# Boulder-Computer-Architecture-Lab/shrewd

Measured on AMD Instinct MI355X. Metric: fault-injection trials/sec (whole node), higher is better.
Workload: dtype int64; 1 GPU; crc32 (RV64, 64618 golden insts), 100000 single-bit x1..x31+pc trials per GPU per step; trials_per_gpu=100000, seed=0x5eed0002, structures=x1-x31,pc, burst=1, lanes_per_wave=32, parallelism=trial-sharded x1, RCCL histogram all-reduce

## Files before the change

### include/fi_debug.h

```cpp
#ifndef SHREWD_FI_DEBUG_H
#define SHREWD_FI_DEBUG_H
#include "fi_engine.h"
#ifdef __cplusplus
extern "C" {
#endif
fi_status fi_debug_decode(fi_engine *e, const uint32_t *raws, uint64_t n, void *out);
fi_status fi_debug_stats(fi_engine *e, uint64_t *out64);
fi_status fi_debug_softfp(int op, int fmt, int rm, const uint64_t *a, const uint64_t *b, const uint64_t *c,
                          uint64_t n, uint64_t *out, uint32_t *fl, int on_device);
fi_status fi_debug_waves(fi_engine *e, uint64_t *out, uint64_t n_waves);
fi_status fi_debug_dispatch_ms(fi_engine *e, float *ms, uint32_t cap, uint32_t *n);
fi_status fi_debug_dispatch_span_ms(fi_engine *e, float *ms, uint32_t cap, uint32_t *n);
fi_status fi_debug_dispatch_kinds(fi_engine *e, uint32_t *kinds, uint32_t cap, uint32_t *n);
fi_status fi_debug_epochs(fi_engine *e, uint32_t *out16);
fi_status fi_debug_golden_trace(fi_engine *e, void *pre_out, uint64_t pre_cap, uint64_t *n_pre, uint32_t *trace_out,
                                uint64_t trace_cap, uint64_t *n_trace, uint64_t *text_lo);
fi_status fi_debug_translate(const void *pre, uint64_t n_pre, uint64_t text_lo, const uint32_t *trace,
                             uint64_t n_trace, char *out, uint64_t cap, uint64_t *len);
fi_status fi_debug_loop_est(const void *pre, uint64_t n_pre, uint64_t text_lo, const uint32_t *trace,
                            uint64_t n_trace, void *out, uint64_t cap, uint64_t *n);
fi_status fi_debug_translation(fi_engine *e, char *buf, uint64_t cap, uint64_t *len);
fi_status fi_debug_jit_compile(const char *body, const char *arch, void *code, uint64_t cap, uint64_t *len,
                               char *err, uint64_t err_cap);
fi_status fi_debug_jit_build(const char *body, const char *arch, int part, int use_cache, uint64_t *len,
                             int *cached, char *err, uint64_t err_cap);

typedef struct {
    uint64_t regs[32];
    uint64_t left;
    uint32_t lp_cnt, lp_m, lp_n;
    uint32_t lp_ld[4][3];
    uint32_t pad;
} fi_debug_loop;
typedef struct {
    int32_t verdict;
    uint32_t body_proof;
    uint64_t k, fva;
} fi_debug_loop_out;
fi_status fi_debug_loop_outcome(fi_engine *e, const fi_debug_loop *in, uint64_t n, fi_debug_loop_out *out);
#ifdef __cplusplus
}
// ... 3 lines not shown
```

### include/fi_engine.h

```cpp
#ifndef SHREWD_FI_ENGINE_H
#define SHREWD_FI_ENGINE_H

#ifndef __HIPCC_RTC__
#include <stddef.h>
#include <stdint.h>
#endif

#ifdef __cplusplus
extern "C" {
#endif

typedef int32_t fi_status;
#define FI_OK 0
#define FI_E_ARG -1
#define FI_E_NODEVICE -2
#define FI_E_HIP -3
#define FI_E_ELF -4
#define FI_E_STATE -5
#define FI_E_GOLDEN -6

#define FI_MASKED 0
#define FI_SDC 1
#define FI_CRASH 2
#define FI_HANG 3
// ... 69 lines not shown
    uint32_t flags;
    uint32_t epoch_iters;
    uint32_t lanes_per_wave;
    uint32_t resume_lanes;
    uint32_t epochs;
} fi_config;
#define FI_CFG_NO_SNAPSHOT_START 1u
#define FI_CFG_NO_EARLY_EXIT 2u
#define FI_CFG_NO_TRANSLATE 4u
#define FI_CFG_NO_EPOCHS 8u
#define FI_CFG_PACK_RUNS 16u
#define FI_CFG_FIXED_RESUME 32u
#define FI_CFG_NO_SOLO 64u
#define FI_CFG_SOLO_ALL 128u
#define FI_CFG_SIMT 256u
#define FI_CFG_NO_FORWARD 512u
#define FI_CFG_NO_SDC_EXIT 1024u
#define FI_CFG_NO_REDO 2048u
#define FI_CFG_NO_ODD_KERNEL 4096u
#define FI_CFG_JIT_NO_CACHE 8192u
#define FI_CFG_NO_HANG_PROOF 16384u
#define FI_CFG_NO_OVERFLOW 32768u
#define FI_CFG_NO_LOOP_ORDER 65536u

typedef struct {
    uint64_t ninst, ncycles;
    uint32_t exit_code, pad;
    uint64_t stdout_len, stderr_len;
    uint64_t fetch_bytes, data_bytes;
    uint64_t snapshots, snapshot_interval;
    uint64_t snapshot_frames;
    uint64_t translated_blocks;
    uint64_t translated_insts;
    uint64_t translate_us;
} fi_golden_info;

typedef struct {
    uint64_t counts[FI_N_STRUCT][64][FI_N_CLASS];
    uint64_t crash_sub[16];
    uint64_t escape_sub[8];
    uint64_t trials;
    uint64_t guest_insts;
    uint64_t fetch_bytes;
    uint64_t data_bytes;
    uint64_t cow_pages;
    uint64_t device_insts;
// ... 172 lines not shown
```

### shrewd_amd/csrc/fi_engine.cpp

```cpp
#include <hip/hip_runtime.h>

#include <algorithm>
#include <atomic>
#include <chrono>
#include <condition_variable>
#include <memory>
#include <mutex>
#include <thread>
#include <cstdarg>
#include <cstdio>
#include <cstdlib>
#include <cstring>
#include <map>
#include <random>
#include <string>
#include <vector>

#include "fi_capture.h"
#include "fi_checkpoint.h"
#include "fi_debug.h"
#include "fi_site_draw.h"
#include "fi_tick.h"
#include "fi_tick_map.h"
#include "fi_types.h"
// ... 24 lines not shown
                       const unsigned long long *stats, hipStream_t st);
hipError_t launch_hist_stats(const unsigned long long *stats, fi_histogram *h, hipStream_t st);
hipError_t sort_pairs_bytes(uint64_t n, size_t &bytes);
hipError_t launch_pack_runs(const uint64_t *keys, const uint32_t *cnt, uint64_t cap, uint32_t *wrange,
                            uint32_t *n_waves, hipStream_t st);
hipError_t launch_redo_collect(const fi_outcome *out, uint64_t n, uint32_t *idx, uint32_t *cnt,
                               unsigned long long *stats, hipStream_t st);
hipError_t launch_redo_gather(const fi_site *sites, const uint32_t *idx, uint64_t n, fi_site *rsites, uint64_t *keys,
                              uint32_t *perm, hipStream_t st);
hipError_t launch_redo_scatter(const uint32_t *idx, uint64_t n, const fi_outcome *rout, fi_outcome *out,
                               hipStream_t st);
hipError_t launch_capture_init(uint8_t *rows, uint64_t n, uint32_t stride, uint32_t cap, const uint8_t *gold,
                               uint64_t glen, hipStream_t st);
hipError_t launch_capture_finish(uint8_t *rows, uint64_t n, uint32_t stride, uint32_t cap, const fi_stream_len *lens,
                                 uint32_t err, hipStream_t st);
hipError_t launch_surv_keys(const LaneSave *save, const uint32_t *list, const uint32_t *cnt, uint64_t cap,
                            uint64_t text_lo, uint64_t *keys, uint32_t *vals, uint32_t *n_odd, uint32_t solo,
                            uint64_t golden_ninst, uint32_t nb, const LoopEst *loops, uint32_t n_loops,
                            uint64_t hang_cap, hipStream_t st);
hipError_t launch_odd_split(const uint32_t *cnt, const uint32_t *n_odd, uint32_t *split, uint32_t grid,
                            hipStream_t st);
std::string translate_blocks(const std::vector<PreInst> &pre, uint64_t text_lo, const std::vector<uint32_t> &trace,
                             const std::vector<uint64_t> &extra_pcs, std::vector<uint32_t> &leaders_out,
                             uint32_t &n_insts, bool odd_streams, std::vector<LoopEst> *loops_out = nullptr);
std::vector<fi_issue_op> issue_ops_from_trace(const std::vector<PreInst> &pre, const std::vector<uint32_t> &trace);
std::string jit_compile(const std::string &body, const char *arch, std::vector<char> &code, bool &cached, int part,
                        bool use_cache);
bool jit_has_odd(const std::string &body);
bool jit_parallel_ok();
hipError_t sort_pairs(void *tmp, size_t bytes, const uint64_t *kin, uint64_t *kout, const uint32_t *vin,
                      uint32_t *vout, uint64_t n, int end_bit, hipStream_t st);
}

using namespace fi;

static constexpr uint32_t kDefaultLanes = 32;
static constexpr uint32_t kPreTail = 4;
static constexpr uint32_t kDefaultResumeLanes = 8;
static constexpr uint64_t kJitWindowChunk = 131072;

struct JitJob {
    std::string body, arch;
    bool odd = false;
    bool use_cache = true;
    std::vector<char> code[3];
    std::string err;
    bool cached = true;
// ... 1152 lines not shown
            HIPCHK(hipMalloc(&e->d_fw_off, 33 * 4));
            HIPCHK(hipMalloc(&e->d_fw_ev, std::max<size_t>(ev.size(), 1) * 4));
            HIPCHK(hipMemcpy(e->d_fw_off, off.data(), 33 * 4, hipMemcpyHostToDevice));
            if (!ev.empty()) HIPCHK(hipMemcpy(e->d_fw_ev, ev.data(), ev.size() * 4, hipMemcpyHostToDevice));
            e->fw_ok = true;
        }
    }
    st = upload_snaps(e);
    if (st) return st;
    st = build_mem_index(e, mev, live_ok && n_mem <= mem_cap);
    if (st) return st;
    e->golden_unmapped = stats[62] != 0;
    tick_prepare(e, mev, !trace.empty() && n_mem <= mem_cap);

    free_tx(e);
    if (e->cfg.flags & FI_CFG_NO_TRANSLATE) e->tx_status = "disabled (FI_CFG_NO_TRANSLATE)";
    else if (!e->pre_ok) e->tx_status = "golden run rewrites its text";
    else if (!live_ok || trace.empty()) e->tx_status = "golden trace unavailable";
    else {
        const std::vector<uint64_t> pcs;
        std::vector<uint32_t> leaders;
        std::vector<LoopEst> loops;
        uint32_t n_tx = 0;
        std::string body = translate_blocks(pre, e->text_lo, trace, pcs, leaders, n_tx, true, &loops);
        if (n_tx > 24000) {
            leaders.clear();
            loops.clear();
            body = translate_blocks(pre, e->text_lo, trace, pcs, leaders, n_tx, false, &loops);
        }
        if (!loops.empty() && !(e->cfg.flags & FI_CFG_NO_LOOP_ORDER)) {
            HIPCHK(hipMalloc(&e->d_loops, loops.size() * sizeof(LoopEst)));
            HIPCHK(hipMemcpy(e->d_loops, loops.data(), loops.size() * sizeof(LoopEst), hipMemcpyHostToDevice));
            e->n_loops = (uint32_t)loops.size();
        }
        e->tx_body = body;
        hipDeviceProp_t prop;
        HIPCHK(hipGetDeviceProperties(&prop, e->dev));
        if (const char *dump = getenv("SHREWD_FI_DUMP_TX")) {
            if (FILE *f = fopen(dump, "w")) { fputs(body.c_str(), f); fclose(f); }
        }
        if (leaders.empty()) {
            e->tx_status = "nothing to translate (no code run twice)";
        } else if (n_tx > 24000) {
            e->tx_status = "translation too large";
        } else {
            auto j = std::make_shared<JitJob>();
            j->body = body;
            j->arch = prop.gcnArchName;
            j->odd = jit_has_odd(body);
            j->use_cache = !(e->cfg.flags & FI_CFG_JIT_NO_CACHE);
            for (uint32_t h : leaders) pre[h & 0x7FFFFFFFu].flags |= (h >> 31) ? kPreOddLeader : kPreLeader;
// ... 869 lines not shown
    if (trace_out) memcpy(trace_out, e->g_trace.data(), std::min<uint64_t>(trace_cap, e->g_trace.size()) * 4);
    if (n_pre) *n_pre = e->g_pre.size();
    if (n_trace) *n_trace = e->g_trace.size();
    if (text_lo) *text_lo = e->text_lo;
    return FI_OK;
}

fi_status fi_debug_loop_est(const void *pre, uint64_t n_pre, uint64_t text_lo, const uint32_t *trace,
                            uint64_t n_trace, void *out, uint64_t cap, uint64_t *n) {
    if (!pre || !trace) return FI_E_ARG;
    std::vector<PreInst> p((const PreInst *)pre, (const PreInst *)pre + n_pre);
    std::vector<uint32_t> t(trace, trace + n_trace), leaders;
    std::vector<LoopEst> loops;
    uint32_t n_tx = 0;
    (void)translate_blocks(p, text_lo, t, {}, leaders, n_tx, true, &loops);
    static_assert(sizeof(LoopEst) == 16, "LoopEst is 16 bytes (fi_debug.h)");
    if (out) memcpy(out, loops.data(), std::min<uint64_t>(cap, loops.size()) * sizeof(LoopEst));
    if (n) *n = loops.size();
    return FI_OK;
}

fi_status fi_debug_translate(const void *pre, uint64_t n_pre, uint64_t text_lo, const uint32_t *trace,
                             uint64_t n_trace, char *out, uint64_t cap, uint64_t *len) {
    if (!pre || !trace) return FI_E_ARG;
    std::vector<PreInst> p((const PreInst *)pre, (const PreInst *)pre + n_pre);
    std::vector<uint32_t> t(trace, trace + n_trace);
    std::vector<uint32_t> leaders;
    uint32_t n_tx = 0;
    const std::string body = translate_blocks(p, text_lo, t, {}, leaders, n_tx, true);
    if (out && cap) {
        const uint64_t n = std::min<uint64_t>(cap - 1, body.size());
        memcpy(out, body.data(), n);
        out[n] = 0;
    }
    if (len) *len = body.size();
    return FI_OK;
}

fi_status fi_debug_translation(fi_engine *e, char *buf, uint64_t cap, uint64_t *len) {
    if (!e) return FI_E_ARG;
    if (buf && cap) {
        const uint64_t n = std::min<uint64_t>(cap - 1, e->tx_body.size());
        memcpy(buf, e->tx_body.data(), n);
        buf[n] = 0;
    }
    if (len) *len = e->tx_body.size();
    return FI_OK;
}

fi_status fi_debug_stats(fi_engine *e, uint64_t *out64) {
    if (!e || !out64) return FI_E_ARG;
    HIPCHK(hipStreamSynchronize(e->stream));
// ... 105 lines not shown
```

### shrewd_amd/csrc/fi_translate.cpp

```cpp
#include <cstdlib>
#include <cctype>
#include <cstdarg>
#include <cstdio>
#include <algorithm>
#include <cstring>
#include <map>
#include <set>
#include <unordered_map>
#include <string>
#include <vector>

#include "fi_types.h"
#include "rv64_isa.h"

namespace fi {

namespace {

struct Gen {
    const std::vector<PreInst> &pre;
    uint64_t text_lo;
    const std::set<uint32_t> &leaders;
    const std::set<uint32_t> &executed;
    std::string out;
// ... 272 lines not shown
            }
            if (top) entries.insert(header);
            headers.insert(header);
            for (uint32_t v : comp) chain[v].push_back(header);
            auto inner = removed;
            for (uint32_t v : comp) inner.insert({v, header});
            run(comp, false, inner);
        }
    }
};

struct Block {
    uint32_t h0;
    std::vector<uint32_t> insts;
    bool term;
    uint64_t opc = 0;
    std::vector<uint64_t> opcs;
};

}

std::string translate_blocks(const std::vector<PreInst> &pre, uint64_t text_lo, const std::vector<uint32_t> &trace,
                             const std::vector<uint64_t> &extra_pcs, std::vector<uint32_t> &leaders_out,
                             uint32_t &n_insts, bool odd_streams, std::vector<LoopEst> *loops_out) {
    std::set<uint32_t> executed, leaders;
    auto valid = [&](uint32_t h) { return h < pre.size() && (pre[h].flags & kPreValid); };
    std::unordered_map<uint32_t, uint32_t> runs;
    for (size_t i = 0; i < trace.size(); i++) {
        const uint32_t h = trace[i] & 0x7FFFFFFFu;
        if (valid(h)) runs[h]++;
    }
    for (size_t i = 0; i < trace.size(); i++) {
        const uint32_t h = trace[i] & 0x7FFFFFFFu;
        if (!valid(h) || runs[h] < 2) continue;
        executed.insert(h);
        const bool is_ecall = trace[i] & 0x80000000u;
        if (i == 0) leaders.insert(h);
        if (i + 1 < trace.size()) {
            const uint32_t nh = trace[i + 1] & 0x7FFFFFFFu;
            if (is_ecall || nh != h + pre[h].len / 2u) leaders.insert(nh);
        }
    }
    for (auto it = leaders.begin(); it != leaders.end();) {
        if (!executed.count(*it)) it = leaders.erase(it);
        else ++it;
    }
    for (uint32_t h : executed) {
// ... 148 lines not shown
            const Cls k = ocls(pc);
            if (k == C_BR || k == C_JAL || k == C_JALR) { b.term = true; break; }
            pc += pre[okey(pc)].len;
        }
        blocks.push_back(b);
    }
    bool cur_odd = false;
    bool oddon = false;
    std::string SB = "S_", SD = "S_dispatch", SOB = "SO_";

    enum Edge { E_DIRECT, E_DISPATCH, E_OUT };
    auto edge = [&](uint32_t from, uint64_t pc) {
        uint32_t t;
        if (!hof(pc, t)) return E_OUT;
        return S.exits.count({from, t}) ? E_DISPATCH : E_DIRECT;
    };

    Gen g{pre, text_lo, leaders, executed, {}};
    Gen so{pre, text_lo, leaders, executed, {}};
    Gen sq{pre, text_lo, leaders, executed, {}};
    Gen sc{pre, text_lo, leaders, executed, {}};
    constexpr uint32_t kSiteCaches = 8;
    uint32_t n_sites = 0;
    n_insts = 0;
    auto hex = [](uint64_t v) {
        char b[32];
        snprintf(b, sizeof b, "0x%llxULL", (unsigned long long)v);
        return std::string(b);
    };
    auto wgo = [&](uint32_t from, uint64_t pc) {
        const Edge k = edge(from, pc);
        uint32_t t = 0;
        hof(pc, t);
        if (k == E_DIRECT) return "goto B_" + std::to_string(t) + ";";
        return "{ spc = " + hex(pc) + (k == E_DISPATCH ? "; goto tx_dispatch; }" : "; goto tx_out; }");
    };
    const char *cold = "SCOLD";
    auto sgo = [&](uint32_t from, uint64_t pc) {
        if (oddon && (pc & 1))
            return olead.count(pc) ? "goto " + SOB + std::to_string((uint32_t)((pc - text_lo) >> 1)) + ";"
                                   : "{ spc = " + hex(pc) + "; goto S_out; }";
        if (oddon && cur_odd) return "{ spc = " + hex(pc) + "; goto " + SD + "; }";
        const Edge k = edge(from, pc);
        uint32_t t = 0;
        hof(pc, t);
        if (k == E_DIRECT) return "goto " + SB + std::to_string(t) + ";";
        return "{ spc = " + hex(pc) + (k == E_DISPATCH ? "; goto " + SD + "; }" : "; goto S_out; }");
    };
    struct ProofLoad { uint32_t reg, kind, size, pos; int64_t off; uint64_t span; };
    struct HangProof { uint32_t reg, treg; int step; uint32_t m; std::vector<ProofLoad> loads; bool rel = false; };
    std::map<uint32_t, HangProof> hang_proof;
    struct AVal { int k; uint32_t base; int64_t lo, hi; };
    enum { AV_TOP, AV_CNT, AV_BND, AV_IND };
    const int64_t kAvLim = (int64_t)1 << 40;
    auto av_ok = [&](AVal v) { return v.k == AV_BND && v.lo > -kAvLim && v.hi < kAvLim && v.lo <= v.hi ? v : AVal{AV_TOP, 0, 0, 0}; };
    auto av_add = [&](AVal a, AVal b) -> AVal {
        if (a.k != AV_BND || b.k != AV_BND || (a.base && b.base)) return AVal{AV_TOP, 0, 0, 0};
        return av_ok(AVal{AV_BND, a.base | b.base, a.lo + b.lo, a.hi + b.hi});
    };
    auto av_shl = [&](AVal a, int64_t k) -> AVal {
        if (a.k != AV_BND || a.base || a.lo < 0 || k < 0 || k > 20) return AVal{AV_TOP, 0, 0, 0};
        return av_ok(AVal{AV_BND, 0, a.lo << k, a.hi << k});
    };
    auto av_const = [&](int64_t lo, int64_t hi) { return av_ok(AVal{AV_BND, 0, lo, hi}); };
    for (uint32_t H : S.headers) {
        std::vector<uint32_t> cyc;
        bool nested = false;
        for (const auto &kv : S.chain) {
            const auto pos = std::find(kv.second.begin(), kv.second.end(), H);
            if (pos == kv.second.end()) continue;
            if (pos + 1 != kv.second.end()) nested = true;
            cyc.push_back(kv.first);
        }
        if (nested || cyc.empty()) continue;
        const std::set<uint32_t> in(cyc.begin(), cyc.end());
        std::map<uint32_t, const Block *> bl;
        for (const Block &b : blocks)
            if (b.opc == 0 && in.count(b.h0)) bl[b.h0] = &b;
        if (bl.size() != in.size()) continue;
        bool ok = true;
        uint32_t writes[32] = {0};
        std::map<uint32_t, std::vector<uint32_t>> nx;
        uint32_t n_exit = 0, eblk = 0;
        bool exit_on_taken = false;
        for (const auto &kv : bl) {
            const Block &b = *kv.second;
            if (b.insts.empty()) { ok = false; break; }
            auto to = [&](uint64_t pc, bool taken) {
                uint32_t t;
                if (hof(pc, t) && in.count(t) && !S.exits.count({b.h0, t})) nx[b.h0].push_back(t);
                else { n_exit++; eblk = b.h0; exit_on_taken = taken; }
            };
            for (size_t i = 0; i < b.insts.size() && ok; i++) {
                std::string e;
                uint32_t sz;
                int sx;
                const char *cond;
                const PreInst &p = pre[b.insts[i]];
                const uint64_t pc = text_lo + 2ULL * b.insts[i];
                const Cls k = classify(p, e, sz, sx, cond);
                if (k == C_JALR || k == C_STOP || ((k == C_LOAD || k == C_STORE) && in.size() != 1)) ok = false;
                if ((k == C_ALU || k == C_JAL || k == C_LOAD) && p.rd) writes[p.rd]++;
                if (k == C_BR) { to(pc + (int64_t)p.imm, true); to(pc + p.len, false); }
                if (k == C_JAL) to(pc + (int64_t)p.imm, true);
            }
            if (ok && !b.term) to(text_lo + 2ULL * b.insts.back() + pre[b.insts.back()].len, false);
        }
        if (!ok || n_exit != 1) continue;
        const Block &E = *bl[eblk];
        const PreInst &br = pre[E.insts.back()];
        uint32_t reg = 0, treg = 0;
        bool exit_when_zero = false;
        if (br.op == OP_c_beqz || br.op == OP_c_bnez) {
            reg = br.rs1;
            exit_when_zero = (br.op == OP_c_beqz) == exit_on_taken;
        } else if ((br.op == OP_beq || br.op == OP_bne) && (br.rs1 == 0) != (br.rs2 == 0)) {
            reg = br.rs1 ? br.rs1 : br.rs2;
            exit_when_zero = (br.op == OP_beq) == exit_on_taken;
        } else if ((br.op == OP_beq || br.op == OP_bne) && br.rs1 && br.rs2 && br.rs1 != br.rs2) {
            if (writes[br.rs1] == 1 && writes[br.rs2] == 0) { reg = br.rs1; treg = br.rs2; }
            else if (writes[br.rs2] == 1 && writes[br.rs1] == 0) { reg = br.rs2; treg = br.rs1; }
            exit_when_zero = (br.op == OP_beq) == exit_on_taken;
        }
        if (!reg || !exit_when_zero || writes[reg] != 1) continue;
        int step = 0;
        for (size_t i = 0; i + 1 < E.insts.size(); i++) {
            const PreInst &p = pre[E.insts[i]];
            const int a = p.imm < 0 ? -p.imm : p.imm;
            if ((p.op == OP_addi || p.op == OP_c_addi) && p.rd == reg && p.rs1 == reg && (a == 1 || a == 2 || a == 4 || a == 8))
                step = p.imm;
        }
        if (!step) continue;
        std::vector<ProofLoad> loads;
        if (in.size() == 1) {
            AVal av[32];
            for (uint32_t r = 0; r < 32; r++) av[r] = writes[r] ? AVal{AV_TOP, 0, 0, 0} : AVal{AV_BND, r, 0, 0};
            int ind_step[32] = {0};
            for (size_t i = 0; i < E.insts.size(); i++) {
                const PreInst &p = pre[E.insts[i]];
                if ((p.op == OP_addi || p.op == OP_c_addi) && p.rd && p.rd == p.rs1 && p.rd != reg && writes[p.rd] == 1 &&
                    p.imm != 0 && p.imm >= -2048 && p.imm <= 2048) {
                    ind_step[p.rd] = p.imm;
                    av[p.rd] = AVal{AV_IND, p.rd, 0, 0};
                }
            }
            av[reg] = AVal{AV_CNT, 0, 0, 0};
            for (size_t i = 0; i < E.insts.size() && ok; i++) {
                std::string e;
                uint32_t sz;
                int sx;
                const char *cond;
                const PreInst &p = pre[E.insts[i]];
                const Cls k = classify(p, e, sz, sx, cond);
                const AVal A = av[p.rs1], B = av[p.rs2];
                const int64_t imm = p.imm;
                if (k == C_LOAD) {
                    if (A.k == AV_CNT) loads.push_back({reg, 0u, sz, (uint32_t)i, A.lo + imm, 0u});
                    else if (A.k == AV_IND)
                        loads.push_back({A.base, 3u, sz, (uint32_t)i, A.lo + imm, (uint64_t)(uint32_t)ind_step[A.base]});
                    else if (A.k == AV_BND) loads.push_back({A.base, 1u, sz, (uint32_t)i, A.lo + imm, (uint64_t)(A.hi - A.lo)});
                    else ok = false;
                    if (p.rd) av[p.rd] = AVal{AV_TOP, 0, 0, 0};
                    continue;
                }
                if (k == C_STORE) {
                    if (A.k == AV_CNT) loads.push_back({reg, 2u, sz, (uint32_t)i, A.lo + imm, 0u});
                    else if (A.k == AV_IND)
                        loads.push_back({A.base, 4u, sz, (uint32_t)i, A.lo + imm, (uint64_t)(uint32_t)ind_step[A.base]});
                    else ok = false;
                    continue;
                }
                if (!p.rd || (k != C_ALU && k != C_JAL)) continue;
                AVal v{AV_TOP, 0, 0, 0};
                if (k == C_ALU) switch (p.op) {
                case OP_addi: case OP_c_addi: case OP_c_addi4spn: case OP_c_addi16sp:
                    if (A.k == AV_CNT) v = AVal{AV_CNT, 0, A.lo + imm, A.lo + imm};
                    else if (A.k == AV_IND && p.rd == A.base) v = AVal{AV_IND, A.base, A.lo + imm, A.lo + imm};
                    else v = av_add(A, av_const(imm, imm));
                    break;
                case OP_add: case OP_c_add: v = av_add(A, B); break;
                case OP_c_mv: v = B; break;
                case OP_andi: case OP_c_andi: if (imm >= 0) v = av_const(0, imm); break;
                case OP_c_zext_b: v = av_const(0, 0xFF); break;
                case OP_c_zext_h: v = av_const(0, 0xFFFF); break;
                case OP_slli: case OP_c_slli: v = av_shl(A, imm); break;
                case OP_srli: case OP_c_srli: if (imm >= 44 && imm < 64) v = av_const(0, (int64_t)((1ULL << (64 - imm)) - 1)); break;
                case OP_sh1add: v = av_add(av_shl(A, 1), B); break;
                case OP_sh2add: v = av_add(av_shl(A, 2), B); break;
                case OP_sh3add: v = av_add(av_shl(A, 3), B); break;
                case OP_c_li: case OP_lui: v = av_const(imm, imm); break;
                default: break;
                }
                av[p.rd] = v;
            }
            for (const ProofLoad &l : loads)
                if (l.off <= -((int64_t)1 << 31) || l.off >= ((int64_t)1 << 31) || (l.kind < 3 && l.span >= (1u << 20)))
                    ok = false;
            if (!ok || loads.size() > 4) continue;
        }
        std::map<uint32_t, uint32_t> dist;
        std::set<std::pair<uint32_t, uint32_t>> q;
        for (uint32_t t : nx[eblk]) {
            const uint32_t d = (uint32_t)bl[t]->insts.size();
            if (!dist.count(t) || d < dist[t]) { dist[t] = d; q.insert({d, t}); }
        }
        uint32_t m = 0;
        while (!q.empty()) {
            const auto [d, v] = *q.begin();
            q.erase(q.begin());
            if (d != dist[v]) continue;
            if (v == eblk) { m = d; break; }
            for (uint32_t t : nx[v]) {
                const uint32_t nd = d + (uint32_t)bl[t]->insts.size();
                if (!dist.count(t) || nd < dist[t]) { dist[t] = nd; q.insert({nd, t}); }
            }
        }
        if (!m) continue;
// ... 309 lines not shown
        const uint64_t pc0 = cur_odd ? b.opc : g.pc_of(h0);
        const std::string P0 = hex(pc0);
        uint32_t rw = 0;
        for (uint32_t hh : insts) {
            const PreInst &p = pre[hh];
            if ((p.flags & kPreRs1) && p.rs1) rw |= 1u << p.rs1;
            if ((p.flags & kPreRs2) && p.rs2) rw |= 1u << p.rs2;
            if ((p.flags & kPreRd) && p.rd) rw |= 1u << p.rd;
        }
        uint64_t blo = pc0 & ~3ULL, bhi = g.pc_of(insts.empty() ? h0 : insts.back()) + 6;
        if (cur_odd) {
            blo = ~0ULL; bhi = 0;
            for (uint32_t hh : insts) {
                blo = std::min<uint64_t>(blo, g.pc_of(hh) & ~3ULL);
                bhi = std::max<uint64_t>(bhi, g.pc_of(hh) + 7);
            }
        }
        g.put("B_%u: { // pc 0x%llx, %u insts\n", h0, (unsigned long long)pc0, n);
        if (cur_odd)
            so_.put("%s%u: { // pc 0x%llx (odd)\n", SOB.c_str(), (uint32_t)((pc0 - text_lo) >> 1),
                    (unsigned long long)pc0);
        else
            sboth(sfmt("%s%u: { // pc 0x%llx, %u insts\n", SB.c_str(), h0, (unsigned long long)pc0, n));
        if (!cur_odd && S.headers.count(h0)) {
            std::string rw_, rs_, rc_;
            for (uint32_t x : leaders) {
                auto it = S.chain.find(x);
                if (it == S.chain.end() || x == h0) continue;
                const auto &ch = it->second;
                const auto pos = std::find(ch.begin(), ch.end(), h0);
                if (pos == ch.end()) continue;
                const uint32_t next = (pos + 1 != ch.end()) ? *(pos + 1) : x;
                const std::string clr = S.headers.count(next) ? "" : "etgt = 0xFFFFFFFFu; ";
                const std::string sclr = S.headers.count(next) ? "" : "eon = 0; ";
                rw_ += "case " + std::to_string(x) + ": " + clr + "goto B_" + std::to_string(next) + "; ";
                rs_ += "case " + std::to_string(x) + ": " + sclr + "goto " + SB + std::to_string(next) + "; ";
                const std::string chk = (!oddon && next == x && !is_cp(x))
                    ? sfmt("if (SOVER(%uu)) { spc = %s; bst = 1u; goto S_out; } ", run_len[x], hex(g.pc_of(x)).c_str())
                    : std::string();
                rc_ += "case " + std::to_string(x) + ": " + sclr + chk + "goto " + SB + std::to_string(next) + "; ";
            }
            const char *fmt = "  if (etgt != 0xFFFFFFFFu) { if (etgt == %uu) etgt = 0xFFFFFFFFu; "
                              "else switch (etgt) { %sdefault: break; } }\n";
            const char *sfm = "  ETGT_OPAQUE(); if (__builtin_expect(eon != 0, 0)) { if (etgt == %uu) eon = 0; "
                              "else switch (etgt) { %sdefault: break; } }\n";
            g.put(fmt, h0, rw_.c_str());
// ... 12 lines not shown
                (uint32_t)(bhi - text_lo), P0.c_str());
        if (!oddon && is_cp(h0)) sc.put("  if (SOVER(%uu)) { spc = %s; bst = 1u; goto S_out; }\n", run_len[h0], P0.c_str());
        uint32_t k_st = 0, k_xt = 0, k_fb = 0, k_db = 0;
        auto commit = [&](uint32_t st, uint32_t xt, uint32_t fb, uint32_t db) {
            if (!st) return std::string();
            std::string r = "{ const uint32_t mm_ = mine ? 0xFFFFFFFFu : 0u; lst += " + std::to_string(st) + "u & mm_; ";
            if (xt) r += "lxt += " + std::to_string(xt) + "u & mm_; ";
            if (fb) r += "lfb += " + std::to_string(fb) + "u & mm_; ";
            if (db) r += "ldb += " + std::to_string(db) + "u & mm_; ";
            return r + "wst = uni32(wst + " + std::to_string(st) + "u); } ";
        };
        auto scommit = [&](uint32_t st, uint32_t xt, uint32_t fb, uint32_t db) {
            if (!st) return std::string();
            std::string r = "SADD(" + std::to_string(st) + "u); ";
            if (xt) r += "xt += " + std::to_string(xt) + "u; ";
            if (fb) r += "fb += " + std::to_string(fb) + "u; ";
            if (db) r += "db += " + std::to_string(db) + "u; ";
            return r;
        };
        for (uint32_t i = 0; i < n; i++) {
            const PreInst &p = pre[insts[i]];
            const uint64_t pc = cur_odd ? b.opcs[i] : g.pc_of(insts[i]);
            const uint64_t ft = pc + p.len;
            std::string e;
            uint32_t sz;
            int sx;
            const char *cond;
            const Cls k = classify(p, e, sz, sx, cond);
            const std::string A = Gen::R(p.rs1), B = Gen::R(p.rs2);
            char immb[48];
            snprintf(immb, sizeof immb, "((uint64_t)(int64_t)%dLL)", p.imm);
            const std::string pcb = hex(pc), ftb = hex(ft);
            const uint32_t xt = (p.flags & kPreStraddle) ? 1 : 0;
            const std::string leave_here = "{ " + commit(k_st, k_xt, k_fb, k_db) + "spc = " + pcb + "; goto tx_out; }";
            const std::string sleave_here = "{ " + scommit(k_st, k_xt, k_fb, k_db) + "spc = " + pcb + "; goto S_out; }";
            switch (k) {
            case C_ALU: {
                const std::string v = subst(e, A, B, immb, pcb);
                if (p.rd) {
                    g.put("  TXSET(%u, %s);\n", p.rd, v.c_str());
                    sboth(sfmt("  SX(%u, %s);\n", p.rd, v.c_str()));
                }
                break;
            }
            case C_NOP:
                break;
            case C_LOAD:
                g.put("  { uint8_t *p_; const bool ok_ = tx_probe(m, %s + %s, %uu, false, p_, tx);\n", A.c_str(), immb, sz);
                g.put("    if (TXB(mine && !ok_)) %s\n", leave_here.c_str());
                {
                    const std::string pl = sfmt("  { uint8_t *p_; bool pv_; if (SCOND(!tx_probe_ld(m, %s + %s, %uu, p_, pv_))) %s\n",
                                                A.c_str(), immb, sz, sleave_here.c_str());
                    so_.out += pl;
                    if (!oddon) {
                        if (S.chain.count(h0) && n_sites < kSiteCaches) {
                            const uint32_t i = n_sites++;
                            sc.put("  { uint8_t *p_; bool pv_; const uint64_t ea_ = %s + %s, vp_ = ea_ >> 12;\n"
                                   "    if (%s(vp_ != CV%u)) { const uint64_t e_ = tlb_find(m, vp_); if (SCOND(!e_)) %s "
                                   "SC_SET(%u, vp_, e_); }\n", A.c_str(), immb, cold, i, sleave_here.c_str(), i);
                            if (sz > 1)
                                sc.put("    if (%s(((uint32_t)ea_ & 4095u) > %uu)) %s\n", cold, 4096u - sz, sleave_here.c_str());
                            sc.put("    p_ = SC_PTR(%u, ea_); pv_ = SC_PRIV(%u);\n", i, i);
                        } else {
                            sc.out += pl;
                        }
                    }
                }
                if (p.rd) {
                    g.put("    p_ = ok_ ? p_ : const_cast<uint8_t *>(zp);\n");
                    sboth(sfmt("    uint64_t v_; if (SPRIV(pv_)) v_ = *(const g_%s *)p_; else v_ = tx_sload(p_, %uu);\n",
                               gtype(sz), sz));
                    if (sx) {
                        g.put("    TXSET(%u, (int64_t)(int%d_t)*(const g_%s *)p_); }\n", p.rd, sx, gtype(sz));
                        sboth(sfmt("    X%u = (uint64_t)(int64_t)(int%d_t)v_; }\n", p.rd, sx));
                    } else {
                        g.put("    TXSET(%u, *(const g_%s *)p_); }\n", p.rd, gtype(sz));
                        sboth(sfmt("    X%u = v_; }\n", p.rd));
                    }
                } else {
                    g.put("  }\n");
                    sboth("  }\n");
                }
                break;
            case C_STORE:
                g.put("  { uint8_t *p_; const bool ok_ = tx_probe(m, %s + %s, %uu, true, p_, tx);\n", A.c_str(), immb, sz);
                g.put("    if (TXB(mine && !ok_)) %s\n", leave_here.c_str());
                g.put("    p_ = (mine && ok_) ? p_ : sink; *(g_%s *)p_ = (%s)%s; }\n", gtype(sz), ltype(sz), B.c_str());
                so_.put("  { uint8_t *p_; const uint64_t ea_ = %s + %s; const uint32_t cs_ = tx_probe_st(m, ea_, %uu, "
                       "p_, tx); if (SCOND(!cs_)) %s\n", A.c_str(), immb, sz, sleave_here.c_str());
                so_.put("    const bool chg_ = SCOND(cs_ & 2u) && SUNI((uint64_t)*(g_%s *)p_) != (uint64_t)(%s)%s;\n", gtype(sz),
                        ltype(sz), B.c_str());
                so_.put("    *(g_%s *)p_ = (%s)%s;\n", gtype(sz), ltype(sz), B.c_str());
                so_.put("    if (SCOND(chg_)) { TXCODE(ea_, %uu); if (SCOND(ea_ < %s && ea_ + %uu > %s)) { %sspc = %s; "
                       "goto S_out; } } }\n", sz, hex(bhi).c_str(), sz, ftb.c_str(),
// ... 60 lines not shown
                g.put("    %s\n", commit(k_st + 1, k_xt + xt, k_fb + p.len, k_db).c_str());
                g.put("    const uint64_t t0_ = rdl64<kNL>(t_, __ffsll((unsigned long long)gmr) - 1);\n");
                g.put("    if (TXB(mine && t_ != t0_)) { dpc = t_; jdiv = mine; goto tx_out; }\n");
                g.put("    spc = uni64(t0_); goto tx_dispatch; }\n");
                sboth(sfmt("  { const uint64_t t_ = (%s + (uint64_t)(int64_t)%lldLL) & ~1ULL;\n", A.c_str(), (long long)im));
                if (rd) sboth(sfmt("    SX(%u, %s);\n", rd, ftb.c_str()));
                sboth(sfmt("    %s spc = SUNI(t_); goto %s; }\n", scommit(k_st + 1, k_xt + xt, k_fb + p.len, k_db).c_str(),
                         SD.c_str()));
                break;
            }
            default:
                break;
            }
            k_st += 1; k_xt += xt; k_fb += p.len; k_db += (k == C_LOAD || k == C_STORE) ? sz : 0;
        }
        if (!b.term) {
            const uint64_t nxt = cur_odd ? (n ? b.opcs[n - 1] + pre[insts[n - 1]].len : pc0)
                                         : n ? g.pc_of(insts[n - 1]) + pre[insts[n - 1]].len : pc0;
            g.put("  %s %s\n", commit(k_st, k_xt, k_fb, k_db).c_str(), wgo(h0, nxt).c_str());
            sboth(sfmt("  %s %s\n", scommit(k_st, k_xt, k_fb, k_db).c_str(), sgo(h0, nxt).c_str()));
        }
        g.put("}\n");
        sboth("}\n");
        if (cur_odd) g.out.swap(g_keep);
    }
    if (oddon) g.out.swap(g_mode);
    }
    cur_odd = false;
    leaders_out.assign(leaders.begin(), leaders.end());
    for (uint64_t pc : olead) leaders_out.push_back(0x80000000u | okey(pc));
    std::string sc_head;
    sc_head += "#undef SADD\n#undef SOVER\n#undef SDONE\n#define SADD(n_) (brem -= (n_))\n"
               "#define SOVER(n_) __builtin_expect(brem < (n_), 0)\n#define SDONE() (bud - brem)\n"
               "#define SCOLD(x) __builtin_expect(!!(x), 0)\n";
    for (uint32_t i = 0; i < kSiteCaches; i++) sc_head += sfmt("  uint64_t CV%u, CP%u; uint32_t CQ%u;\n", i, i, i);
    sc_head += "S_entry:\n";
    for (uint32_t i = 0; i < kSiteCaches; i++) sc_head += sfmt("  CV%u = ~0ULL; CP%u = 0; CQ%u = 0;\n", i, i, i);
    sc_head += "  goto S_dispatch;\n";
    auto hoist = [](std::string t) {
        for (const auto &[from, to] : std::vector<std::pair<std::string, std::string>>{
                 {"uint8_t *p_; ", ""}, {"bool pv_; ", ""}, {"uint64_t v_; ", ""},
                 {", vp_ = ea_ >> 12;", "; vp_ = ea_ >> 12;"}, {"const uint64_t ea_ = ", "ea_ = "},
                 {"const uint64_t e_ = ", "e_ = "}, {"const uint64_t t_ = ", "t_ = "},
                 {"const uint64_t t0_ = ", "t0_ = "}, {"const uint64_t off_ = ", "off_ = "},
                 {"const uint32_t cs_ = ", "cs_ = "}, {"const bool chg_ = ", "chg_ = "},
                 {"const bool ok_ = ", "ok_ = "}, {"const bool c_ = ", "c_ = "},
                 {"const uint64_t tk_ = ", "tk_ = "}, {"const uint32_t mm_ = ", "mm_ = "}}) {
            for (size_t at = t.find(from); at != std::string::npos; at = t.find(from, at + to.size()))
                t.replace(at, from.size(), to);
        }
        return t;
    };
    return g.out + FI_TX_SPLIT + so.out + FI_TX_SPLIT + sq.out + FI_TX_SPLIT + sc_head + hoist(sc.out);
}

}
```

### shrewd_amd/fi.py

```python
from __future__ import annotations

import ctypes as C
import os
from typing import Iterable, Sequence

import numpy as np

from . import build as _build

FI_OK, FI_E_ARG, FI_E_NODEVICE, FI_E_HIP, FI_E_ELF, FI_E_STATE, FI_E_GOLDEN = 0, -1, -2, -3, -4, -5, -6
CLASS_NAMES = ["masked", "sdc", "crash", "hang", "detected", "escape"]
CRASH_NAMES = {1: "panic_unknown_inst", 2: "panic_illegal_inst", 3: "panic_page_fault",
               4: "fatal_syscall_range", 5: "fatal_syscall_unimpl", 6: "fatal_proxy", 7: "abort_fd_assert",
               8: "sigtrap", 9: "fatal_stack_limit", 10: "panic_amo_line", 11: "abort_sc_line", 12: "panic_se_handler",
               13: "panic_m5op", 14: "abort_vset_sew"}
ESCAPE_NAMES = {1: "inst", 2: "syscall", 3: "csr", 4: "host", 5: "resource", 6: "undefined", 7: "timing"}
TICK_ESCAPE_NAMES = {1: "after_noncounting_tick", 2: "pc_straddle_first_fetch", 3: "pc_word_and_alignment",
                     4: "pc_aligned_mid_decode", 5: "pc_two_values", 6: "pc_on_fault_attempt",
                     7: "pc_macro_op_access", 8: "reads_curtick"}
CPU_ATOMIC, CPU_TIMING = 0, 1
TICK_MAPS = {"host": 0, "device": 1}
TICK_CONTRACTS = {"numinst": 0, "literal": 1}
HANG_NAMES = {1: "max_insts", 2: "m5_quiesce"}
END_NAMES = {0: "exit", 1: "m5_exit", 2: "m5_fail"}
# ... 77 lines not shown
    _fields_ = [("device", C.c_int32), ("private_pages", C.c_uint32), ("hang_factor_x16", C.c_uint32),
                ("max_trials_per_launch", C.c_uint32), ("snapshot_interval", C.c_uint32), ("flags", C.c_uint32),
                ("epoch_iters", C.c_uint32), ("lanes_per_wave", C.c_uint32),
                ("resume_lanes", C.c_uint32), ("epochs", C.c_uint32)]


CFG_NO_SNAPSHOT_START = 1
CFG_NO_EARLY_EXIT = 2
CFG_NO_TRANSLATE = 4
CFG_NO_EPOCHS = 8
CFG_PACK_RUNS = 16
CFG_FIXED_RESUME = 32
CFG_NO_SOLO = 64
CFG_SOLO_ALL = 128
CFG_SIMT = 256
CFG_NO_FORWARD = 512
CFG_NO_SDC_EXIT = 1024
CFG_NO_REDO = 2048
CFG_NO_ODD_KERNEL = 4096
CFG_JIT_NO_CACHE = 8192
CFG_NO_HANG_PROOF = 16384
CFG_NO_OVERFLOW = 32768
CFG_NO_LOOP_ORDER = 65536


class GoldenInfo(C.Structure):
    _fields_ = [("ninst", C.c_uint64), ("ncycles", C.c_uint64), ("exit_code", C.c_uint32), ("pad", C.c_uint32),
                ("stdout_len", C.c_uint64), ("stderr_len", C.c_uint64), ("fetch_bytes", C.c_uint64),
                ("data_bytes", C.c_uint64), ("snapshots", C.c_uint64), ("snapshot_interval", C.c_uint64),
                ("snapshot_frames", C.c_uint64), ("translated_blocks", C.c_uint64),
                ("translated_insts", C.c_uint64), ("translate_us", C.c_uint64)]


class IssueParams(C.Structure):
    _fields_ = [("issue_width", C.c_uint32), ("dispatch_width", C.c_uint32), ("commit_width", C.c_uint32),
                ("iq_entries", C.c_uint32), ("rob_entries", C.c_uint32), ("load_latency", C.c_uint32),
                ("priority_to_shadow", C.c_uint32), ("fu_count", C.c_uint32 * 6)]


class IssueStats(C.Structure):
    _fields_ = [("ops", C.c_uint64), ("cycles", C.c_uint64), ("shadow_available", C.c_uint64),
                ("shadow_not_available", C.c_uint64), ("shadow_same_fu", C.c_uint64),
                ("shadow_not_same_fu", C.c_uint64), ("class_available", C.c_uint64 * 12),
                ("class_not_available", C.c_uint64 * 12)]

    def as_dict(self) -> dict:
# ... 134 lines not shown
        L.fi_run_sites.argtypes = [vp, vp, C.c_uint64, vp, vp]
        L.fi_run_sites_capture.argtypes = [vp, vp, C.c_uint64, C.c_uint32, vp, vp, vp, vp, vp]
        L.fi_run_trials_device.argtypes = [vp, C.c_uint64, C.c_uint64, vp, vp, vp]
        L.fi_sync.argtypes = [vp]
        L.fi_last_kernel_ms.restype = C.c_double
        L.fi_last_kernel_ms.argtypes = [vp]
        L.fi_debug_decode.argtypes = [vp, vp, C.c_uint64, vp]
        L.fi_debug_loop_outcome.argtypes = [vp, vp, C.c_uint64, vp]
        L.fi_kernel_timer_reset.argtypes = [vp]
        L.fi_get_config.argtypes = [vp, C.POINTER(_Config)]
        L.fi_debug_stats.argtypes = [vp, vp]
        L.fi_debug_softfp.argtypes = [C.c_int, C.c_int, C.c_int, vp, vp, vp, C.c_uint64, vp, vp, C.c_int]
        L.fi_debug_crypto.argtypes = [C.c_int, vp, vp, C.c_uint64, vp, C.c_int]
        L.fi_kernel_timer_read.argtypes = [vp, C.POINTER(C.c_double), C.POINTER(C.c_uint32)]
        L.fi_debug_waves.argtypes = [vp, vp, C.c_uint64]
        L.fi_debug_epochs.argtypes = [vp, vp]
        L.fi_debug_dispatch_ms.argtypes = [vp, vp, C.c_uint32, C.POINTER(C.c_uint32)]
        L.fi_debug_dispatch_kinds.argtypes = [vp, vp, C.c_uint32, C.POINTER(C.c_uint32)]
        L.fi_debug_dispatch_span_ms.argtypes = [vp, vp, C.c_uint32, C.POINTER(C.c_uint32)]
        L.fi_debug_golden_trace.argtypes = [vp, vp, C.c_uint64, C.POINTER(C.c_uint64), vp, C.c_uint64,
                                            C.POINTER(C.c_uint64), C.POINTER(C.c_uint64)]
        L.fi_debug_translate.argtypes = [vp, C.c_uint64, C.c_uint64, vp, C.c_uint64, C.c_char_p, C.c_uint64,
                                         C.POINTER(C.c_uint64)]
        L.fi_debug_translation.argtypes = [vp, C.c_char_p, C.c_uint64, C.POINTER(C.c_uint64)]
        L.fi_issue_default_params.argtypes = [C.POINTER(IssueParams)]
        L.fi_issue_model_run.argtypes = [vp, C.c_uint64, C.POINTER(IssueParams), vp, C.POINTER(IssueStats)]
        L.fi_set_issue_model.argtypes = [vp, C.POINTER(IssueParams)]
        L.fi_shadow_map.argtypes = [vp, vp, C.c_uint64, C.POINTER(C.c_uint64), C.POINTER(IssueStats)]
        L.fi_timing_default_params.argtypes = [C.POINTER(TimingParams)]
        L.fi_timing_model_run.argtypes = [vp, C.c_uint64, C.POINTER(TimingParams), vp, C.POINTER(TimingStats)]
        L.fi_set_cpu_model.argtypes = [vp, C.c_int, C.POINTER(TimingParams)]
        L.fi_tick_golden.argtypes = [vp, C.POINTER(TickInfo)]
        L.fi_tick_trace.argtypes = [vp, vp, vp, C.c_uint64, C.POINTER(C.c_uint64)]
        L.fi_sample_tick_sites.argtypes = [vp, C.c_uint64, C.c_uint64, vp]
        L.fi_map_tick_sites.argtypes = [vp, vp, C.c_uint64, vp, vp, vp]
        L.fi_run_tick_sites.argtypes = [vp, vp, C.c_uint64, vp, vp]
        L.fi_run_tick_trials.argtypes = [vp, C.c_uint64, C.c_uint64, vp, vp]
        L.fi_set_tick_map.argtypes = [vp, C.c_int]
        L.fi_set_tick_contract.argtypes = [vp, C.c_int]
        L.fi_map_tick_sites_device.argtypes = [vp, vp, C.c_uint64, C.c_uint64, vp, vp, vp, vp]
        L.fi_run_tick_trials_device.argtypes = [vp, C.c_uint64, C.c_uint64, vp, vp, vp]
        L.fi_translate_status.restype = C.c_char_p
        L.fi_translate_status.argtypes = [vp]
        _lib = L
    return _lib

# ... 530 lines not shown
```

Baseline: 24.11 million trials/s.

## Prefetch next-iteration loads in single-block loops of translated code

Adds a load-ahead transform to the JIT translator. For single-block loops whose loads use an induction register with a constant step and which contain no stores, the generated code loads the next iteration's value (ea+step) into a held register and tags it with the expected address. The next iteration hits that held value, which hides global-memory latency across the loop back-edge. The abstract-interpretation walk is factored into a shared helper, and a config flag can disable the feature. The cost is extra registers per site, an extra load that may go unused, and possible increased register pressure in the JIT kernel.

```diff
diff --git a/include/fi_debug.h b/include/fi_debug.h
--- a/include/fi_debug.h
+++ b/include/fi_debug.h
@@ -17,6 +17,8 @@
                                 uint64_t trace_cap, uint64_t *n_trace, uint64_t *text_lo);
 fi_status fi_debug_translate(const void *pre, uint64_t n_pre, uint64_t text_lo, const uint32_t *trace,
                              uint64_t n_trace, char *out, uint64_t cap, uint64_t *len);
+fi_status fi_debug_translate_flags(const void *pre, uint64_t n_pre, uint64_t text_lo, const uint32_t *trace,
+                                   uint64_t n_trace, uint32_t flags, char *out, uint64_t cap, uint64_t *len);
 fi_status fi_debug_loop_est(const void *pre, uint64_t n_pre, uint64_t text_lo, const uint32_t *trace,
                             uint64_t n_trace, void *out, uint64_t cap, uint64_t *n);
 fi_status fi_debug_translation(fi_engine *e, char *buf, uint64_t cap, uint64_t *len);
diff --git a/include/fi_engine.h b/include/fi_engine.h
--- a/include/fi_engine.h
+++ b/include/fi_engine.h
@@ -115,6 +115,7 @@
 #define FI_CFG_NO_HANG_PROOF 16384u
 #define FI_CFG_NO_OVERFLOW 32768u
 #define FI_CFG_NO_LOOP_ORDER 65536u
+#define FI_CFG_NO_LOAD_AHEAD 131072u
 
 typedef struct {
     uint64_t ninst, ncycles;
diff --git a/shrewd_amd/csrc/fi_engine.cpp b/shrewd_amd/csrc/fi_engine.cpp
--- a/shrewd_amd/csrc/fi_engine.cpp
+++ b/shrewd_amd/csrc/fi_engine.cpp
@@ -70,7 +70,8 @@
                             hipStream_t st);
 std::string translate_blocks(const std::vector<PreInst> &pre, uint64_t text_lo, const std::vector<uint32_t> &trace,
                              const std::vector<uint64_t> &extra_pcs, std::vector<uint32_t> &leaders_out,
-                             uint32_t &n_insts, bool odd_streams, std::vector<LoopEst> *loops_out = nullptr);
+                             uint32_t &n_insts, bool odd_streams, std::vector<LoopEst> *loops_out = nullptr,
+                             bool load_ahead = true);
 std::vector<fi_issue_op> issue_ops_from_trace(const std::vector<PreInst> &pre, const std::vector<uint32_t> &trace);
 std::string jit_compile(const std::string &body, const char *arch, std::vector<char> &code, bool &cached, int part,
                         bool use_cache);
@@ -1269,11 +1270,12 @@
         std::vector<uint32_t> leaders;
         std::vector<LoopEst> loops;
         uint32_t n_tx = 0;
-        std::string body = translate_blocks(pre, e->text_lo, trace, pcs, leaders, n_tx, true, &loops);
+        const bool ahead = !(e->cfg.flags & FI_CFG_NO_LOAD_AHEAD);
+        std::string body = translate_blocks(pre, e->text_lo, trace, pcs, leaders, n_tx, true, &loops, ahead);
         if (n_tx > 24000) {
             leaders.clear();
             loops.clear();
-            body = translate_blocks(pre, e->text_lo, trace, pcs, leaders, n_tx, false, &loops);
+            body = translate_blocks(pre, e->text_lo, trace, pcs, leaders, n_tx, false, &loops, ahead);
         }
         if (!loops.empty() && !(e->cfg.flags & FI_CFG_NO_LOOP_ORDER)) {
             HIPCHK(hipMalloc(&e->d_loops, loops.size() * sizeof(LoopEst)));
@@ -2189,12 +2191,18 @@
 
 fi_status fi_debug_translate(const void *pre, uint64_t n_pre, uint64_t text_lo, const uint32_t *trace,
                              uint64_t n_trace, char *out, uint64_t cap, uint64_t *len) {
+    return fi_debug_translate_flags(pre, n_pre, text_lo, trace, n_trace, 0, out, cap, len);
+}
+
+fi_status fi_debug_translate_flags(const void *pre, uint64_t n_pre, uint64_t text_lo, const uint32_t *trace,
+                                   uint64_t n_trace, uint32_t flags, char *out, uint64_t cap, uint64_t *len) {
     if (!pre || !trace) return FI_E_ARG;
     std::vector<PreInst> p((const PreInst *)pre, (const PreInst *)pre + n_pre);
     std::vector<uint32_t> t(trace, trace + n_trace);
     std::vector<uint32_t> leaders;
     uint32_t n_tx = 0;
-    const std::string body = translate_blocks(p, text_lo, t, {}, leaders, n_tx, true);
+    const std::string body = translate_blocks(p, text_lo, t, {}, leaders, n_tx, true, nullptr,
+                                              !(flags & FI_CFG_NO_LOAD_AHEAD));
     if (out && cap) {
         const uint64_t n = std::min<uint64_t>(cap - 1, body.size());
         memcpy(out, body.data(), n);
diff --git a/shrewd_amd/csrc/fi_translate.cpp b/shrewd_amd/csrc/fi_translate.cpp
--- a/shrewd_amd/csrc/fi_translate.cpp
+++ b/shrewd_amd/csrc/fi_translate.cpp
@@ -318,7 +318,7 @@
 
 std::string translate_blocks(const std::vector<PreInst> &pre, uint64_t text_lo, const std::vector<uint32_t> &trace,
                              const std::vector<uint64_t> &extra_pcs, std::vector<uint32_t> &leaders_out,
-                             uint32_t &n_insts, bool odd_streams, std::vector<LoopEst> *loops_out) {
+                             uint32_t &n_insts, bool odd_streams, std::vector<LoopEst> *loops_out, bool load_ahead) {
     std::set<uint32_t> executed, leaders;
     auto valid = [&](uint32_t h) { return h < pre.size() && (pre[h].flags & kPreValid); };
     std::unordered_map<uint32_t, uint32_t> runs;
@@ -513,6 +513,7 @@
     Gen sc{pre, text_lo, leaders, executed, {}};
     constexpr uint32_t kSiteCaches = 8;
     uint32_t n_sites = 0;
+    std::map<uint32_t, uint32_t> ahead_sites;
     n_insts = 0;
     auto hex = [](uint64_t v) {
         char b[32];
@@ -554,6 +555,73 @@
         return av_ok(AVal{AV_BND, 0, a.lo << k, a.hi << k});
     };
     auto av_const = [&](int64_t lo, int64_t hi) { return av_ok(AVal{AV_BND, 0, lo, hi}); };
+    struct RunOff { bool ok = true, stores = false; std::vector<ProofLoad> loads; };
+    auto runoff_walk = [&](const Block &E, const uint32_t *writes, uint32_t reg) {
+        RunOff ro;
+        AVal av[32];
+        for (uint32_t r = 0; r < 32; r++) av[r] = writes[r] ? AVal{AV_TOP, 0, 0, 0} : AVal{AV_BND, r, 0, 0};
+        int ind_step[32] = {0};
+        for (size_t i = 0; i < E.insts.size(); i++) {
+            const PreInst &p = pre[E.insts[i]];
+            if ((p.op == OP_addi || p.op == OP_c_addi) && p.rd && p.rd == p.rs1 && p.rd != reg && writes[p.rd] == 1 &&
+                p.imm != 0 && p.imm >= -2048 && p.imm <= 2048) {
+                ind_step[p.rd] = p.imm;
+                av[p.rd] = AVal{AV_IND, p.rd, 0, 0};
+            }
+        }
+        if (reg) av[reg] = AVal{AV_CNT, 0, 0, 0};
+        for (size_t i = 0; i < E.insts.size(); i++) {
+            std::string e;
+            uint32_t sz;
+            int sx;
+            const char *cond;
+            const PreInst &p = pre[E.insts[i]];
+            const Cls k = classify(p, e, sz, sx, cond);
+            const AVal A = av[p.rs1], B = av[p.rs2];
+            const int64_t imm = p.imm;
+            if (k == C_LOAD) {
+                if (A.k == AV_CNT) ro.loads.push_back({reg, 0u, sz, (uint32_t)i, A.lo + imm, 0u});
+                else if (A.k == AV_IND)
+                    ro.loads.push_back({A.base, 3u, sz, (uint32_t)i, A.lo + imm, (uint64_t)(uint32_t)ind_step[A.base]});
+                else if (A.k == AV_BND) ro.loads.push_back({A.base, 1u, sz, (uint32_t)i, A.lo + imm, (uint64_t)(A.hi - A.lo)});
+                else ro.ok = false;
+                if (p.rd) av[p.rd] = AVal{AV_TOP, 0, 0, 0};
+                continue;
+            }
+            if (k == C_STORE) {
+                ro.stores = true;
+                if (A.k == AV_CNT) ro.loads.push_back({reg, 2u, sz, (uint32_t)i, A.lo + imm, 0u});
+                else if (A.k == AV_IND)
+                    ro.loads.push_back({A.base, 4u, sz, (uint32_t)i, A.lo + imm, (uint64_t)(uint32_t)ind_step[A.base]});
+                else ro.ok = false;
+                continue;
+            }
+            if (!p.rd || (k != C_ALU && k != C_JAL)) continue;
+            AVal v{AV_TOP, 0, 0, 0};
+            if (k == C_ALU) switch (p.op) {
+            case OP_addi: case OP_c_addi: case OP_c_addi4spn: case OP_c_addi16sp:
+                if (A.k == AV_CNT) v = AVal{AV_CNT, 0, A.lo + imm, A.lo + imm};
+                else if (A.k == AV_IND && p.rd == A.base) v = AVal{AV_IND, A.base, A.lo + imm, A.lo + imm};
+                else v = av_add(A, av_const(imm, imm));
+                break;
+            case OP_add: case OP_c_add: v = av_add(A, B); break;
+            case OP_c_mv: v = B; break;
+            case OP_andi: case OP_c_andi: if (imm >= 0) v = av_const(0, imm); break;
+            case OP_c_zext_b: v = av_const(0, 0xFF); break;
+            case OP_c_zext_h: v = av_const(0, 0xFFFF); break;
+            case OP_slli: case OP_c_slli: v = av_shl(A, imm); break;
+            case OP_srli: case OP_c_srli: if (imm >= 44 && imm < 64) v = av_const(0, (int64_t)((1ULL << (64 - imm)) - 1)); break;
+            case OP_sh1add: v = av_add(av_shl(A, 1), B); break;
+            case OP_sh2add: v = av_add(av_shl(A, 2), B); break;
+            case OP_sh3add: v = av_add(av_shl(A, 3), B); break;
+            case OP_c_li: case OP_lui: v = av_const(imm, imm); break;
+            default: break;
+            }
+            av[p.rd] = v;
+        }
+        return ro;
+    };
+    std::map<uint32_t, int> ahead_at;
     for (uint32_t H : S.headers) {
         std::vector<uint32_t> cyc;
         bool nested = false;
@@ -597,6 +665,15 @@
             }
             if (ok && !b.term) to(text_lo + 2ULL * b.insts.back() + pre[b.insts.back()].len, false);
         }
+        if (load_ahead && ok && in.size() == 1 && !nx[H].empty()) {
+            const Block &L = *bl[H];
+            const RunOff ro = runoff_walk(L, writes, 0);
+            for (const ProofLoad &l : ro.loads) {
+                const PreInst &p = pre[L.insts[l.pos]];
+                if (!ro.stores && l.kind == 3 && p.rs1 == l.reg && p.rd && p.rd != l.reg)
+                    ahead_at[L.insts[l.pos]] = (int)(int32_t)(uint32_t)l.span;
+            }
+        }
         if (!ok || n_exit != 1) continue;
         const Block &E = *bl[eblk];
         const PreInst &br = pre[E.insts.back()];
@@ -624,66 +701,9 @@
         if (!step) continue;
         std::vector<ProofLoad> loads;
         if (in.size() == 1) {
-            AVal av[32];
-            for (uint32_t r = 0; r < 32; r++) av[r] = writes[r] ? AVal{AV_TOP, 0, 0, 0} : AVal{AV_BND, r, 0, 0};
-            int ind_step[32] = {0};
-            for (size_t i = 0; i < E.insts.size(); i++) {
-                const PreInst &p = pre[E.insts[i]];
-                if ((p.op == OP_addi || p.op == OP_c_addi) && p.rd && p.rd == p.rs1 && p.rd != reg && writes[p.rd] == 1 &&
-                    p.imm != 0 && p.imm >= -2048 && p.imm <= 2048) {
-                    ind_step[p.rd] = p.imm;
-                    av[p.rd] = AVal{AV_IND, p.rd, 0, 0};
-                }
-            }
-            av[reg] = AVal{AV_CNT, 0, 0, 0};
-            for (size_t i = 0; i < E.insts.size() && ok; i++) {
-                std::string e;
-                uint32_t sz;
-                int sx;
-                const char *cond;
-                const PreInst &p = pre[E.insts[i]];
-                const Cls k = classify(p, e, sz, sx, cond);
-                const AVal A = av[p.rs1], B = av[p.rs2];
-                const int64_t imm = p.imm;
-                if (k == C_LOAD) {
-                    if (A.k == AV_CNT) loads.push_back({reg, 0u, sz, (uint32_t)i, A.lo + imm, 0u});
-                    else if (A.k == AV_IND)
-                        loads.push_back({A.base, 3u, sz, (uint32_t)i, A.lo + imm, (uint64_t)(uint32_t)ind_step[A.base]});
-                    else if (A.k == AV_BND) loads.push_back({A.base, 1u, sz, (uint32_t)i, A.lo + imm, (uint64_t)(A.hi - A.lo)});
-                    else ok = false;
-                    if (p.rd) av[p.rd] = AVal{AV_TOP, 0, 0, 0};
-                    continue;
-                }
-                if (k == C_STORE) {
-                    if (A.k == AV_CNT) loads.push_back({reg, 2u, sz, (uint32_t)i, A.lo + imm, 0u});
-                    else if (A.k == AV_IND)
-                        loads.push_back({A.base, 4u, sz, (uint32_t)i, A.lo + imm, (uint64_t)(uint32_t)ind_step[A.base]});
-                    else ok = false;
-                    continue;
-                }
-                if (!p.rd || (k != C_ALU && k != C_JAL)) continue;
-                AVal v{AV_TOP, 0, 0, 0};
-                if (k == C_ALU) switch (p.op) {
-                case OP_addi: case OP_c_addi: case OP_c_addi4spn: case OP_c_addi16sp:
-                    if (A.k == AV_CNT) v = AVal{AV_CNT, 0, A.lo + imm, A.lo + imm};
-                    else if (A.k == AV_IND && p.rd == A.base) v = AVal{AV_IND, A.base, A.lo + imm, A.lo + imm};
-                    else v = av_add(A, av_const(imm, imm));
-                    break;
-                case OP_add: case OP_c_add: v = av_add(A, B); break;
-                case OP_c_mv: v = B; break;
-                case OP_andi: case OP_c_andi: if (imm >= 0) v = av_const(0, imm); break;
-                case OP_c_zext_b: v = av_const(0, 0xFF); break;
-                case OP_c_zext_h: v = av_const(0, 0xFFFF); break;
-                case OP_slli: case OP_c_slli: v = av_shl(A, imm); break;
-                case OP_srli: case OP_c_srli: if (imm >= 44 && imm < 64) v = av_const(0, (int64_t)((1ULL << (64 - imm)) - 1)); break;
-                case OP_sh1add: v = av_add(av_shl(A, 1), B); break;
-                case OP_sh2add: v = av_add(av_shl(A, 2), B); break;
-                case OP_sh3add: v = av_add(av_shl(A, 3), B); break;
-                case OP_c_li: case OP_lui: v = av_const(imm, imm); break;
-                default: break;
-                }
-                av[p.rd] = v;
-            }
+            const RunOff ro = runoff_walk(E, writes, reg);
+            ok = ro.ok;
+            loads = ro.loads;
             for (const ProofLoad &l : loads)
                 if (l.off <= -((int64_t)1 << 31) || l.off >= ((int64_t)1 << 31) || (l.kind < 3 && l.span >= (1u << 20)))
                     ok = false;
@@ -1039,6 +1059,23 @@
                     (unsigned long long)pc0);
         else
             sboth(sfmt("%s%u: { // pc 0x%llx, %u insts\n", SB.c_str(), h0, (unsigned long long)pc0, n));
+        std::map<uint32_t, uint32_t> blk_ahead;
+        const size_t sc_at = sc.out.size();
+        if (!oddon && !cur_odd && S.chain.count(h0)) {
+            uint32_t ns = n_sites;
+            for (uint32_t i = 0; i < n && ns < kSiteCaches; i++) {
+                std::string e;
+                uint32_t sz;
+                int sx;
+                const char *cond;
+                const Cls k = classify(pre[insts[i]], e, sz, sx, cond);
+                if (k != C_LOAD && k != C_STORE) continue;
+                if (k == C_LOAD && ahead_at.count(insts[i])) blk_ahead[i] = ns;
+                ns++;
+            }
+            for (const auto &kv : blk_ahead) sc.put("  HT%u = ~0ULL;\n", kv.second);
+            if (!blk_ahead.empty()) sc.put("%s%u_L: ;\n", SB.c_str(), h0);
+        }
         if (!cur_odd && S.headers.count(h0)) {
             std::string rw_, rs_, rc_;
             for (uint32_t x : leaders) {
@@ -1097,6 +1134,8 @@
             const PreInst &p = pre[insts[i]];
             const uint64_t pc = cur_odd ? b.opcs[i] : g.pc_of(insts[i]);
             const uint64_t ft = pc + p.len;
+            const uint32_t i_inst = i;
+            int sc_site = -1;
             std::string e;
             uint32_t sz;
             int sx;
@@ -1130,9 +1169,12 @@
                     if (!oddon) {
                         if (S.chain.count(h0) && n_sites < kSiteCaches) {
                             const uint32_t i = n_sites++;
+                            sc_site = (int)i;
+                            const std::string drop = blk_ahead.count(i_inst) ? sfmt("HT%u = ~0ULL; ", i) : std::string();
                             sc.put("  { uint8_t *p_; bool pv_; const uint64_t ea_ = %s + %s, vp_ = ea_ >> 12;\n"
                                    "    if (%s(vp_ != CV%u)) { const uint64_t e_ = tlb_find(m, vp_); if (SCOND(!e_)) %s "
-                                   "SC_SET(%u, vp_, e_); }\n", A.c_str(), immb, cold, i, sleave_here.c_str(), i);
+                                   "SC_SET(%u, vp_, e_); %s}\n", A.c_str(), immb, cold, i, sleave_here.c_str(), i,
+                                   drop.c_str());
                             if (sz > 1)
                                 sc.put("    if (%s(((uint32_t)ea_ & 4095u) > %uu)) %s\n", cold, 4096u - sz, sleave_here.c_str());
                             sc.put("    p_ = SC_PTR(%u, ea_); pv_ = SC_PRIV(%u);\n", i, i);
@@ -1143,8 +1185,20 @@
                 }
                 if (p.rd) {
                     g.put("    p_ = ok_ ? p_ : const_cast<uint8_t *>(zp);\n");
-                    sboth(sfmt("    uint64_t v_; if (SPRIV(pv_)) v_ = *(const g_%s *)p_; else v_ = tx_sload(p_, %uu);\n",
-                               gtype(sz), sz));
+                    const std::string ld = sfmt("    uint64_t v_; if (SPRIV(pv_)) v_ = *(const g_%s *)p_; else v_ = tx_sload(p_, %uu);\n",
+                                                gtype(sz), sz);
+                    so_.out += ld;
+                    if (!oddon && sc_site >= 0 && blk_ahead.count(i_inst)) {
+                        const int stp = ahead_at[insts[i_inst]];
+                        sc.put("    uint64_t v_; if (HT%d == ea_) v_ = HV%d; else v_ = *(const g_%s *)p_;\n", sc_site, sc_site,
+                               gtype(sz));
+                        sc.put("    if (%s(((uint32_t)ea_ & 4095u) + (uint32_t)%d > %uu)) HT%d = ~0ULL;\n"
+                               "    else { HV%d = *(const g_%s *)(p_ + %d); HT%d = ea_ + (uint64_t)(int64_t)%d; }\n", cold, stp,
+                               4096u - sz, sc_site, sc_site, gtype(sz), stp, sc_site, stp);
+                        ahead_sites[(uint32_t)sc_site] = sz;
+                    } else if (!oddon) {
+                        sc.out += ld;
+                    }
                     if (sx) {
                         g.put("    TXSET(%u, (int64_t)(int%d_t)*(const g_%s *)p_); }\n", p.rd, sx, gtype(sz));
                         sboth(sfmt("    X%u = (uint64_t)(int64_t)(int%d_t)v_; }\n", p.rd, sx));
@@ -1251,6 +1305,11 @@
         }
         g.put("}\n");
         sboth("}\n");
+        if (!blk_ahead.empty()) {
+            const std::string from = sfmt("goto %s%u;", SB.c_str(), h0), to = sfmt("goto %s%u_L;", SB.c_str(), h0);
+            for (size_t at = sc.out.find(from, sc_at); at != std::string::npos; at = sc.out.find(from, at + to.size()))
+                sc.out.replace(at, from.size(), to);
+        }
         if (cur_odd) g.out.swap(g_keep);
     }
     if (oddon) g.out.swap(g_mode);
@@ -1263,6 +1322,8 @@
                "#define SOVER(n_) __builtin_expect(brem < (n_), 0)\n#define SDONE() (bud - brem)\n"
                "#define SCOLD(x) __builtin_expect(!!(x), 0)\n";
     for (uint32_t i = 0; i < kSiteCaches; i++) sc_head += sfmt("  uint64_t CV%u, CP%u; uint32_t CQ%u;\n", i, i, i);
+    for (const auto &kv : ahead_sites)
+        sc_head += sfmt("  %s HV%u; uint64_t HT%u;\n", kv.second == 8 ? "uint64_t" : "uint32_t", kv.first, kv.first);
     sc_head += "S_entry:\n";
     for (uint32_t i = 0; i < kSiteCaches; i++) sc_head += sfmt("  CV%u = ~0ULL; CP%u = 0; CQ%u = 0;\n", i, i, i);
     sc_head += "  goto S_dispatch;\n";
diff --git a/shrewd_amd/fi.py b/shrewd_amd/fi.py
--- a/shrewd_amd/fi.py
+++ b/shrewd_amd/fi.py
@@ -123,6 +123,7 @@
 CFG_NO_HANG_PROOF = 16384
 CFG_NO_OVERFLOW = 32768
 CFG_NO_LOOP_ORDER = 65536
+CFG_NO_LOAD_AHEAD = 131072
 
 
 class GoldenInfo(C.Structure):
@@ -303,6 +304,8 @@
                                             C.POINTER(C.c_uint64), C.POINTER(C.c_uint64)]
         L.fi_debug_translate.argtypes = [vp, C.c_uint64, C.c_uint64, vp, C.c_uint64, C.c_char_p, C.c_uint64,
                                          C.POINTER(C.c_uint64)]
+        L.fi_debug_translate_flags.argtypes = [vp, C.c_uint64, C.c_uint64, vp, C.c_uint64, C.c_uint32, C.c_char_p,
+                                               C.c_uint64, C.POINTER(C.c_uint64)]
         L.fi_debug_translation.argtypes = [vp, C.c_char_p, C.c_uint64, C.POINTER(C.c_uint64)]
         L.fi_issue_default_params.argtypes = [C.POINTER(IssueParams)]
         L.fi_issue_model_run.argtypes = [vp, C.c_uint64, C.POINTER(IssueParams), vp, C.POINTER(IssueStats)]
```

Measured after the change: 25.47 million trials/s (median of 6 runs). 1.06x the previous value.
